# r4dl/StopThePop-Rasterization

Measured on AMD Instinct MI355X. Metric: fwd+bwd frames/sec at 1920×1080, 1M Gaussians; PSNR vs reference, higher is better.
Workload: dtype f32

## Files before the change

stopthepop-rasterization_amd/csrc/stp_render_hier.inc:

```
#include "stp_internal.h"
#include "stp_blend.h"

namespace stp {

#ifdef STP_HIER_STATS
static __device__ unsigned long long g_hier_stats[16];
#if defined(STP_INST_MODE) && STP_INST_MODE == 2 && STP_INST_MID == 8
extern "C" int stp_debug_hier_stats(unsigned long long* out16)
{
    hipError_t e = hipMemcpyFromSymbol(out16, HIP_SYMBOL(g_hier_stats), sizeof(unsigned long long) * 16);
    unsigned long long z[16] = {};
    (void)hipMemcpyToSymbol(HIP_SYMBOL(g_hier_stats), z, sizeof(z));
    return (int)e;
}
#endif
#endif

namespace {

#ifndef STP_BWD_WIN
#define STP_BWD_WIN 256
#endif
#ifndef STP_BWD_RING
#define STP_BWD_RING 512
#endif
#ifndef STP_BWD_WAVES
#define STP_BWD_WAVES 3
#endif
#ifndef STP_FWD_WAVES
#define STP_FWD_WAVES 5
#endif
constexpr int BWD_WIN = STP_BWD_WIN;
constexpr int BWD_RING = STP_BWD_RING;

#ifndef STP_FIFO_GROUPS
#define STP_FIFO_GROUPS 4
#endif
constexpr int FIFO_GROUPS = STP_FIFO_GROUPS;
#ifndef STP_HF_CAP
#define STP_HF_CAP 32
#endif
constexpr int HF_CAP = STP_HF_CAP;

struct HierLds {
    static __host__ __device__ constexpr size_t tail_key() { return 0; }
    static __host__ __device__ constexpr size_t tail_id() { return 16 * 64 * 4; }
    static __host__ __device__ constexpr size_t new_key() { return 2 * 16 * 64 * 4; }
    static __host__ __device__ constexpr size_t new_id() { return 2 * 16 * 64 * 4 + 16 * 32 * 4; }
    static __host__ __device__ constexpr size_t mid_key() { return 2 * 16 * 64 * 4 + 2 * 16 * 32 * 4; }
    static __host__ __device__ constexpr size_t mid_id(int MID) { return mid_key() + 64 * (size_t)MID * 4; }
    static __host__ __device__ constexpr size_t fifo(int MID) { return mid_key() + 2 * 64 * (size_t)MID * 4; }
    static __host__ __device__ constexpr size_t rays(int MID) { return fifo(MID) + 16 * (size_t)FIFO_GROUPS * 16 * 4; }
    static __host__ __device__ constexpr size_t mid_rays(int MID) { return rays(MID) + 4 * 2 * 8 * 4; }
    static __host__ __device__ constexpr size_t fwd_total(int MID) { return mid_rays(MID) + 64 * 4 * 4; }
    static __host__ __device__ constexpr size_t hfifo(int MID) { return fwd_total(MID); }
    static __host__ __device__ constexpr size_t acc(int MID) { return fwd_total(MID); }
    static __host__ __device__ constexpr size_t tag(int MID) { return acc(MID) + 9 * (size_t)BWD_WIN * 8; }
    static __host__ __device__ constexpr size_t dirty(int MID) { return tag(MID) + (size_t)BWD_WIN * 4; }
    static __host__ __device__ constexpr size_t ring(int MID) { return dirty(MID) + (size_t)BWD_WIN * 4; }
    static __host__ __device__ constexpr size_t ring_cs(int MID) { return ring(MID) + (size_t)BWD_RING * 4; }
    static __host__ __device__ constexpr size_t wave_mask(int MID) { return ring_cs(MID) + (size_t)BWD_RING * 4; }
    static __host__ __device__ constexpr size_t total(int MID, int mode) { return mode == 1 ? wave_mask(MID) + 16 : hfifo(MID) + 64 * (size_t)HF_CAP * 4; }
};

__device__ __forceinline__ int hier_remap_tile(int wg, int n_wg)
{
    const int q = n_wg >> 3, r = n_wg & 7;
    const int xcd = wg & 7, k = wg >> 3;
    return (xcd < r ? xcd * (q + 1) : r * (q + 1) + (xcd - r) * q) + k;
}

constexpr int MODE_FWD = 0, MODE_BWD = 1, MODE_FWD_RECORD = 2, MODE_FWD_DEPTH = 3;

template <int HEAD, int MID, bool CULL, int MODE, bool FRCP>
__global__ void __launch_bounds__(256, MODE == MODE_BWD ? STP_BWD_WAVES : (HEAD == 4 && MID == 8 && FRCP) ? STP_FWD_WAVES : 4) render_hier_kernel(const RenderArgs a)
{
    constexpr bool FRESH_QUAD = MODE != MODE_BWD && HEAD == 4 && MID == 8 && FRCP && STP_FWD_WAVES >= 5 && CULL;
    constexpr bool BACKWARD = MODE == MODE_BWD;
    constexpr bool RECORD = MODE == MODE_FWD_RECORD;
    constexpr bool DEPTHVIZ = MODE == MODE_FWD_DEPTH;
    constexpr bool USE_POS = true;
    extern __shared__ __attribute__((aligned(16))) char smem[];
    constexpr int OLDN = (MID - 4) / 4;

    const int lane = (int)(threadIdx.x & 63);
    const int w = __builtin_amdgcn_readfirstlane((int)(threadIdx.x >> 6));
    const int s = lane >> 4;
    const int x = lane & 15;
    const int m = x >> 2;
    const int q = x & 3;

    const int rows = a.ty1 - a.ty0;
    const int t = a.tile_order ? (int)a.tile_order[blockIdx.x] : hier_remap_tile((int)blockIdx.x, a.gx * rows);
    const int tile_x = t % a.gx, tile_y = a.ty0 + t / a.gx;
    const uint2 range = a.ranges[tile_y * a.gx + tile_x];
    if constexpr (BACKWARD) {
        if (a.flag_mode == 1 && a.tile_flags[tile_y * a.gx + tile_x] == 0u) return;
    }

    const int cx = tile_x * TILE + 4 * s, cy = tile_y * TILE + 4 * w;
    const int px = cx + 2 * (m & 1) + (q & 1), py = cy + 2 * (m >> 1) + (q >> 1);
    const bool inside = px < a.W && py < a.H;
    bool active = inside;
    if constexpr (!BACKWARD) {
        if (range.y <= range.x) {
            if (inside) {
                const size_t N = (size_t)a.W * a.H, pid = (size_t)a.W * py + px;
                a.final_T[pid] = 1.0f;
                if constexpr (RECORD) a.n_contrib[pid] = 0u;
                if constexpr (DEPTHVIZ) { a.out_color[pid] = 0.0f; a.out_color[N + pid] = 1.0f; }
                else { a.out_color[pid] = a.bg[0]; a.out_color[N + pid] = a.bg[1]; a.out_color[2 * N + pid] = a.bg[2]; }
            }
            return;
        }
    }
    if constexpr (MODE == MODE_FWD || MODE == MODE_FWD_RECORD) {
        const int n = (int)(range.y - range.x);
        if (a.fused_gather && n <= TS_SMALL) {
            tile_sort_gather_lds(a.gather, reinterpret_cast<uint64_t*>(smem), tile_y * a.gx + tile_x, range, n, (int)threadIdx.x);
            __threadfence_block();
            __syncthreads();
        }
    }

    const int st = w * 4 + s;
    auto fresh_lane = [&]() __attribute__((always_inline)) -> int {
        int l;
        asm volatile("v_mbcnt_lo_u32_b32 %0, -1, 0\n\tv_mbcnt_hi_u32_b32 %0, -1, %0" : "=v"(l));
        return l;
    };
#define STP_ROW_VIEW(L)                                                                                                  \
    const int lrow_ = (L);                                               \
    const int x = lrow_ & 15;                                                                                            \
    const int st_r = w * 4 + (lrow_ >> 4);                                                                               \
    float* const tk = reinterpret_cast<float*>(smem + HierLds::tail_key()) + st_r * 64;                                  \
    int* const ti = reinterpret_cast<int*>(smem + HierLds::tail_id()) + st_r * 64;                                       \
    float* const nk = reinterpret_cast<float*>(smem + HierLds::new_key()) + st_r * 32;                                   \
    int* const ni = reinterpret_cast<int*>(smem + HierLds::new_id()) + st_r * 32;                                        \
    int* const fifo = reinterpret_cast<int*>(smem + HierLds::fifo(MID)) + st_r * FIFO_GROUPS * 16;
    struct QuadView { int q; float* mk; int* mi; int* hfifo; };
#define STP_QUAD_VIEW(L)                                                                                                 \
    const int lquad_ = (L);                                              \
    const int q = lquad_ & 3;                                                                                            \
    const uint32_t qi_ = (uint32_t)(w * 16) + ((uint32_t)lquad_ >> 2);                                                   \
    const uint32_t qmid_ = (MID & (MID - 1)) == 0 ? qi_ << __builtin_ctz(MID) : qi_ * (uint32_t)MID;  \
    float* const mk = reinterpret_cast<float*>(smem + HierLds::mid_key()) + qmid_;                                       \
    int* const mi = reinterpret_cast<int*>(smem + HierLds::mid_id(MID)) + qmid_;                                         \
    float* const mray = reinterpret_cast<float*>(smem + HierLds::mid_rays(MID)) + (qi_ << 2);                            \
    int* const hfifo = reinterpret_cast<int*>(smem + HierLds::hfifo(MID)) + (qi_ << __builtin_ctz(HF_CAP));             \
    const QuadView qv{q, mk, mi, hfifo}; (void)qv; (void)mray;

    const float3 cam = make_float3(a.cam[0], a.cam[1], a.cam[2]);
    const float3 pix_dir = view_ray(a.inv_vp, cam, (float)px, (float)py, a.W, a.H);
    if (q == 0) {
        float* const mray = reinterpret_cast<float*>(smem + HierLds::mid_rays(MID)) + (st * 4 + m) * 4;
        const float3 md = view_ray(a.inv_vp, cam, (float)cx + 0.5f + 2.0f * (float)(m & 1), (float)cy + 0.5f + 2.0f * (float)(m >> 1), a.W, a.H);
        mray[0] = md.x; mray[1] = md.y; mray[2] = md.z; mray[3] = 0.0f;
    }
#define STP_STAGE_VIEW(L)                                                                                                \
    const int lstage_ = (L);                                             \
    const int half = lstage_ >> 5, e = lstage_ & 31;                                                                           \
    const int sxA = tile_x * TILE + 4 * (2 * half), sxB = sxA + 4;                                                       \
    float* const tray = reinterpret_cast<float*>(smem + HierLds::rays(MID)) + (w * 2 + half) * 8;                        \
    float* const nkA = reinterpret_cast<float*>(smem + HierLds::new_key()) + (w * 4 + 2 * half) * 32;                    \
    int* const niA = reinterpret_cast<int*>(smem + HierLds::new_id()) + (w * 4 + 2 * half) * 32;
    {
    STP_STAGE_VIEW(lane)
    if (e == 0) {
        const float3 tA = view_ray(a.inv_vp, cam, (float)sxA + 1.5f, (float)cy + 1.5f, a.W, a.H);
        const float3 tB = view_ray(a.inv_vp, cam, (float)sxB + 1.5f, (float)cy + 1.5f, a.W, a.H);
        tray[0] = tA.x; tray[1] = tA.y; tray[2] = tA.z; tray[3] = 0.0f;
        tray[4] = tB.x; tray[5] = tB.y; tray[6] = tB.z; tray[7] = 0.0f;
    }
    }
    wave_sync();

    unsigned long long* const acc = reinterpret_cast<unsigned long long*>(smem + HierLds::acc(MID));
    int* const tag = reinterpret_cast<int*>(smem + HierLds::tag(MID));
    int* const dirty = reinterpret_cast<int*>(smem + HierLds::dirty(MID));
    int* const ring = reinterpret_cast<int*>(smem + HierLds::ring(MID));
    int* const ring_cs = reinterpret_cast<int*>(smem + HierLds::ring_cs(MID));
    unsigned int* const wave_mask = reinterpret_cast<unsigned int*>(smem + HierLds::wave_mask(MID));
    const float4* const eA = a.entA + range.x;
    const float4* const eB = a.entB + range.x;
    const float4* const eC = a.entC + range.x;
    const float4* const eD = a.entD + range.x;
    const float4* const eF = a.entF + range.x;
    const int list_last = max((int)(range.y - range.x) - 1, 0);
    auto ent_row = [&](const float4* base, int pos) __attribute__((always_inline)) -> float4 {
        return *reinterpret_cast<const float4*>(reinterpret_cast<const char*>(base) + ((uint32_t)pos << 4));
    };
    int staged = 0;
    int ccount = 0;
    auto to_id = [&](int v) __attribute__((always_inline)) -> int {
        if constexpr (!USE_POS) return v;
        else {
            int r = ring[v & (BWD_RING - 1)];
            const bool old = v >= 0 && v < staged - BWD_RING;
            if (__builtin_expect(__any(old), 0)) {
                if (old) r = (int)a.point_list[range.x + min(v, list_last)];
            }
            return v < 0 ? -1 : r;
        }
    };
    if constexpr (BACKWARD) {
        for (int i = (int)threadIdx.x; i < BWD_WIN; i += 256) {
            tag[i] = -1;
            dirty[i] = 0;
#pragma unroll
            for (int k = 0; k < 9; k++) acc[k * BWD_WIN + i] = 0ull;
        }
        __syncthreads();
    }

    char* const log_wave = RECORD ? log_wave_slice(a.blend_log, tile_y * a.gx + tile_x, __builtin_amdgcn_readfirstlane(w), a.log_depth) : nullptr;
    const uint32_t log_cap2 = 2u * (uint32_t)a.log_depth;
    const uint32_t log_lane16 = (uint32_t)lane << LOG_PIECE_SHIFT;
    uint32_t log_j2 = 0u;
    auto log_append = [&](bool upd, int pay) __attribute__((always_inline)) {
        *reinterpret_cast<log_t*>(log_wave + log_record_offset<false>(min(log_j2, log_cap2), log_lane16)) = (log_t)pay;
        log_j2 += upd ? 2u : 0u;
    };
    auto log_records = [&]() __attribute__((always_inline)) -> int { return (int)(log_j2 >> 1); };
    auto log_finish = [&]() __attribute__((always_inline)) {};

    Window<HEAD> head;
    if constexpr (BACKWARD) head.init(); else head.init_padded();
    FwdPixel fp;
    BwdPixel bp;
    if constexpr (BACKWARD) init_bwd_pixel(bp, a, inside, px, py);
    else init_fwd_pixel(fp);

    int n_tail = 0;
    int n_mid = 0;
    int mid_pending = 0;

    float wave_md = 0.0f;
    if constexpr (BACKWARD) {
        wave_md = fmaxf(fmaxf(fabsf(bp.dL_dpix[0]), fabsf(bp.dL_dpix[1])), fabsf(bp.dL_dpix[2]));
#pragma unroll
        for (int off = 32; off > 0; off >>= 1) wave_md = fmaxf(wave_md, __shfl_xor(wave_md, off));
        if (lane == 0) wave_mask[w] = __float_as_uint(wave_md);
        __syncthreads();
        wave_md = fmaxf(fmaxf(__uint_as_float(wave_mask[0]), __uint_as_float(wave_mask[1])),
                        fmaxf(__uint_as_float(wave_mask[2]), __uint_as_float(wave_mask[3])));
        __syncthreads();
    }
    int md_exp = 0;
    if (wave_md > 0.0f && wave_md < 3.0e38f) (void)frexpf(wave_md, &md_exp);
    const double fx_scale = ldexp(1.0, 31 - md_exp), fx_inv = ldexp(1.0, md_exp - 31);
    const float fx_cap = ldexpf(1.0f, min(md_exp + 20, 126));
    auto accumulate = [&](int pos, int id, const float (&g_in)[9]) __attribute__((always_inline)) {
        float g[9];
#pragma unroll
        for (int k = 0; k < 9; k++) g[k] = g_in[k];
        const unsigned long long here = __ballot(1);
        bool mine = true;
        if (((here >> (lane & ~3)) & 0xFull) == 0xFull) {
            const int p0 = quad_bcast_i<0>(pos), p1 = quad_bcast_i<1>(pos), p2 = quad_bcast_i<2>(pos), p3 = quad_bcast_i<3>(pos);
            if (p0 == p1 && p0 == p2 && p0 == p3) {
#pragma unroll
                for (int k = 0; k < 9; k++) {
                    g[k] += __int_as_float(__builtin_amdgcn_mov_dpp(__float_as_int(g[k]), 0xB1, 0xF, 0xF, true));
                    g[k] += __int_as_float(__builtin_amdgcn_mov_dpp(__float_as_int(g[k]), 0x4E, 0xF, 0xF, true));
                }
                mine = q == 0;
            }
        }
        if (!mine) return;
        int cs = -1;
        if (pos >= staged - BWD_RING) cs = ring_cs[pos & (BWD_RING - 1)];
        float gmax = fabsf(g[0]);
#pragma unroll
        for (int k = 1; k < 9; k++) gmax = fmaxf(gmax, fabsf(g[k]));
        if (cs >= 0 && tag[cs] == pos && gmax < fx_cap) {
#pragma unroll
            for (int k = 0; k < 9; k++) {
                const double t = fma((double)g[k], fx_scale, 6755399441055744.0);
                const long long qv = __double_as_longlong(t) - 0x4338000000000000ll;
                atomicAdd(&acc[k * BWD_WIN + cs], (unsigned long long)qv);
            }
            dirty[cs] = 1;
        } else {
#pragma unroll
            for (int k = 0; k < 9; k++) atomicAdd(grad_slot(a, id, k), g[k]);
        }
    };
    auto flush_slot = [&](int cs, int first, int last) __attribute__((always_inline)) {
        if (dirty[cs]) {
            const int old_id = to_id(tag[cs]);
            for (int k = first; k < last; k++) {
                const long long v = (long long)acc[k * BWD_WIN + cs];
                acc[k * BWD_WIN + cs] = 0ull;
                if (v != 0) atomicAdd(grad_slot(a, old_id, k), (float)((double)v * fx_inv));
            }
        }
    };
    auto flush_all = [&]() __attribute__((always_inline)) {
        __syncthreads();
        for (int cs = (int)threadIdx.x; cs < BWD_WIN; cs += 256) flush_slot(cs, 0, 9);
    };

    int front_key = -1;
    float front_col[3] = {0.0f, 0.0f, 0.0f};
    FrontData front_fd{};
    int front_gid = -1;
    auto refresh_front = [&]() __attribute__((always_inline)) {
        if (active && head.num > 0 && head.id[0] != front_key) {
            front_key = head.id[0];
            if constexpr (BACKWARD) {
                front_gid = to_id(front_key);
                front_fd = load_front(a, front_gid);
            } else {
                front_gid = to_id(front_key);
#pragma unroll
                for (int ch = 0; ch < 3; ch++) front_col[ch] = a.features[3 * (size_t)front_gid + ch];
            }
        }
    };
    auto blend_front = [&]() __attribute__((always_inline)) {
        if (!active) { head.num--; return; }
        bool ok;
        if constexpr (BACKWARD) {
            float g[9];
            if (head.id[0] != front_key) refresh_front();
            ok = blend_backward_terms(bp, a, px, py, front_fd, head.store[0], g);
            if (ok) accumulate(head.id[0], front_gid, g);
        } else {
            if (head.id[0] != front_key) refresh_front();
            ok = blend_forward_c(fp, front_col, head.store[0]);
            if constexpr (RECORD) {
                log_append(ok, head.id[0]);
            }
        }
        if (!ok) { active = false; head.num--; return; }
        head.pop();
    };

    float pend_w = 0.0f;
    float pend_c[3] = {0.0f, 0.0f, 0.0f};
    float depth_acc = 0.0f;
    auto pop_forward = [&]() __attribute__((always_inline)) {
#pragma unroll
        for (int ch = 0; ch < 3; ch++) fp.C[ch] = fmaf(pend_w, pend_c[ch], fp.C[ch]);
        const float alpha0 = head.store[0];
        const float test_T = fp.T * (1.0f - alpha0);
        const bool doing = active && !(head.depth[0] < 0.0f);
        const bool upd = doing && !(test_T < T_THRESHOLD);
        const int pay = head.id[0];
        const float4 colr = *reinterpret_cast<const float4*>(reinterpret_cast<const char*>(eF) + ((uint32_t)pay << 4));
        pend_c[0] = colr.x; pend_c[1] = colr.y; pend_c[2] = colr.z;
        pend_w = upd ? alpha0 * fp.T : 0.0f;
        if constexpr (DEPTHVIZ) depth_acc += upd ? head.depth[0] * alpha0 * fp.T : 0.0f;
        fp.T = upd ? test_T : fp.T;
        if constexpr (RECORD) {
            log_append(upd, pay);
        }
        active = active && (upd || !doing);
    };

    auto feed_one = [&](int cid, float3 p0, float3 p1, float3 p2, float4 co, float2 xy) __attribute__((always_inline)) {
        const float depth = depth_along_ray<FRCP>(p0, p1, p2, pix_dir);
        const float dx = xy.x - (float)px, dy = xy.y - (float)py;
        const float power = blend_power(dx, dy, co);
        if constexpr (BACKWARD) {
            if (!active || depth < 0.0f) return;
            if (power > 0.0f) return;
            const float G = exp_blend(power);
            const float alpha = fminf(0.99f, co.w * G);
            if (alpha < ALPHA_THRESHOLD) return;
            head.insert(depth, cid, G);
        } else {
            const float G = exp_blend(power);
            const float alpha = fminf(0.99f, co.w * G);
            const bool pass = active && cid != -1 && !(depth < 0.0f) && !(power > 0.0f) && !(alpha < ALPHA_THRESHOLD);
            head.insert_if(pass, depth, cid, alpha);
        }
    };

    auto feed4_from = [&](const int fid) __attribute__((always_inline)) {
        int pf = 0;
        float4 c0 = make_float4(0, 0, 0, 0), c1 = c0, c2 = c0, co = c0;
        float2 xy = make_float2(0, 0);
        float4 eAq = c0, eBq = c0, eCq = c0, eDq = c0;
        if constexpr (BACKWARD) {
            const int gid_f = to_id(fid);
            if (fid != -1) {
                c0 = a.cov3D_inv[3 * (size_t)gid_f + 0];
                c1 = a.cov3D_inv[3 * (size_t)gid_f + 1];
                c2 = a.cov3D_inv[3 * (size_t)gid_f + 2];
                co = a.conic_opacity[gid_f];
                xy = a.means2D[gid_f];
            }
        } else {
            pf = min(max(fid, 0), list_last);
            eAq = ent_row(eA, pf); eBq = ent_row(eB, pf); eCq = ent_row(eC, pf); eDq = ent_row(eD, pf);
        }
#define STP_FEED(I)                                                                                                     \
    {                                                                                                                   \
                                                                            \
        if constexpr (BACKWARD) { if (head.num >= HEAD) blend_front(); }                                                \
        else pop_forward();                                                                                             \
        const int cid = quad_bcast_i<I>(BACKWARD ? fid : pf);                                                           \
        if constexpr (!BACKWARD) {          \
            if constexpr (I == 0) {                   \
                eDq.w = fid < 0 ? 0.0f : eDq.w;                                                                         \
                dpp_hazard_guard_on(eDq.w);                             \
            } else dpp_hazard_guard();                                                                                  \
            const float depth = depth_along_ray_quad_ent<I, FRCP>(eAq, eBq, eCq, pix_dir);                              \
            const float dx = quad_sub<I>(eCq.y, (float)px), dy = quad_sub<I>(eCq.z, (float)py);                         \
            const float power = blend_power_quad<I>(dx, dy, eDq);                                                       \
            const float alpha = min_099(quad_mul<I>(eDq.w, exp_blend(power)));                                          \
            const bool pass = active && !(depth < 0.0f) && !(power > 0.0f) && !(alpha < ALPHA_THRESHOLD);               \
            head.replace_front(pass, pass ? depth : -FLT_MAX, cid, alpha);                                              \
        } else if (cid != -1) {                                                                                         \
            const float3 b0 = make_float3(quad_bcast<I>(c0.x), quad_bcast<I>(c0.y), quad_bcast<I>(c0.z));               \
            const float3 b1 = make_float3(quad_bcast<I>(c1.x), quad_bcast<I>(c1.y), quad_bcast<I>(c1.z));               \
            const float3 b2 = make_float3(quad_bcast<I>(c2.x), quad_bcast<I>(c2.y), quad_bcast<I>(c2.z));               \
            const float4 bco = make_float4(quad_bcast<I>(co.x), quad_bcast<I>(co.y), quad_bcast<I>(co.z), quad_bcast<I>(co.w)); \
            const float2 bxy = make_float2(quad_bcast<I>(xy.x), quad_bcast<I>(xy.y));                                   \
            feed_one(cid, b0, b1, b2, bco, bxy);                                                                        \
        }                                                                                                               \
// ... 491 lines not shown
```

stopthepop-rasterization_amd/csrc/stp_tilesort.h:

```cpp
#pragma once

#include "stp_device.h"

namespace stp {

constexpr int TS_SMALL = 1024;

struct EntryGather {
    uint64_t* keys;
    uint32_t* point_list;
    const float4* gpack;
    const float* features;
    int gx;
    int cull_mask;
    float4* entA; float4* entB; float4* entC; float4* entD; float4* entF;
};

__device__ __forceinline__ void write_entry(const EntryGather& a, size_t i, int id, int tile)
{
    const float4* __restrict__ gp = a.gpack + 4 * (size_t)id;
    const float4 pa = gp[0], pb = gp[1], pc = gp[2], pd = gp[3];
    const float3 col = make_float3(a.features[3 * (size_t)id], a.features[3 * (size_t)id + 1], a.features[3 * (size_t)id + 2]);
    a.entA[i] = pa;
    a.entB[i] = pb;
    a.entC[i] = make_float4(pc.x, pc.y, pc.z, __int_as_float(id));
    a.entD[i] = pd;
    float spare = 0.0f;
    if (a.cull_mask) spare = __uint_as_float(subtile_mask(a.cull_mask, pd, make_float2(pc.y, pc.z), tile % a.gx, tile / a.gx));
    a.entF[i] = make_float4(col.x, col.y, col.z, spare);
}

__device__ __forceinline__ void tile_sort_gather_lds(const EntryGather& a, uint64_t* s_key, int tile, uint2 range, int n, int tid)
{
    uint64_t* const keys = a.keys + range.x;
    uint32_t* const list = a.point_list + range.x;
    int m = 2;
    while (m < n) m <<= 1;
    const uint64_t tile_bits = keys[0] & 0xFFFFFFFF00000000ull;
    for (int i = tid; i < m; i += 256) {
        s_key[i] = i < n ? ((keys[i] << 32) | list[i]) : ~0ull;
    }
    __syncthreads();
    for (int k = 2; k <= m; k <<= 1)
        for (int j = k >> 1; j > 0; j >>= 1) {
            for (int c = tid; c < (m >> 1); c += 256) {
                const int lo = ((c & ~(j - 1)) << 1) | (c & (j - 1));
                const int hi = lo | j;
                const bool up = (lo & k) == 0;
                const uint64_t x = s_key[lo], y = s_key[hi];
                if ((x > y) == up) { s_key[lo] = y; s_key[hi] = x; }
            }
            const int j_next = j > 1 ? (j >> 1) : k;
            const bool last = j == 1 && k == m;
            if (j > 64 || j_next > 64 || last) __syncthreads();
            else wave_sync();
        }
    for (int i = tid; i < n; i += 256) {
        const uint64_t k = s_key[i];
        const int id = (int)(uint32_t)k;
        keys[i] = tile_bits | (k >> 32);
        list[i] = (uint32_t)id;
        if (a.gpack) write_entry(a, (size_t)range.x + i, id, tile);
    }
}

}
```

stopthepop-rasterization_amd/csrc/stp_tilesort.hip:

```cpp
#include "stp_internal.h"
#include "stp_device.h"
#include "stp_tilesort.h"
#include <rocprim/block/block_radix_sort.hpp>

namespace stp {

namespace {

constexpr int TS_CAP = 4096;
#ifndef STP_GATHER_WAVES
#define STP_GATHER_WAVES 6
#endif

struct TileSortArgs {
    const uint2* ranges;
    uint64_t* keys_scratch;
    uint32_t* list_scratch;
    int id_passes;
    int tile0;
    const uint32_t* tile_order;
    EntryGather e;
};

template <int IPT> struct TileRadix {
    using Sort = rocprim::block_radix_sort<uint32_t, 256, IPT, uint32_t>;
    template <class WriteEntry>
    static __device__ __forceinline__ void run(typename Sort::storage_type& st, uint64_t* keys, uint32_t* list, int n, int tid, WriteEntry&& write_entry_at)
    {
        const uint64_t tile_bits = keys[0] & 0xFFFFFFFF00000000ull;
        uint32_t k[IPT], v[IPT];
#pragma unroll
        for (int j = 0; j < IPT; j++) {
            const int i = tid * IPT + j;
            k[j] = i < n ? (uint32_t)keys[i] : 0xFFFFFFFFu;
            v[j] = i < n ? list[i] : 0xFFFFFFFFu;
        }
        __syncthreads();
        Sort().sort_to_striped(k, v, st, 0, 32);
#pragma unroll
        for (int j = 0; j < IPT; j++) {
            const int i = j * 256 + tid;
            if (i < n) {
                keys[i] = tile_bits | k[j];
                list[i] = v[j];
                write_entry_at(i, (int)v[j]);
            }
        }
    }
};

template <int CAP, int MIN_N>
__global__ void __launch_bounds__(256, (CAP == TS_SMALL ? STP_GATHER_WAVES : 4)) tile_sort_gather_kernel(const TileSortArgs a)
{
    using Radix8 = TileRadix<8>;
    using Radix16 = TileRadix<16>;
    constexpr size_t RADIX_BYTES = CAP == TS_CAP ? (sizeof(typename Radix16::Sort::storage_type) > sizeof(typename Radix8::Sort::storage_type) ? sizeof(typename Radix16::Sort::storage_type) : sizeof(typename Radix8::Sort::storage_type)) : 0;
    constexpr size_t RAW_BYTES = RADIX_BYTES > sizeof(uint64_t) * CAP ? RADIX_BYTES : sizeof(uint64_t) * CAP;
    __shared__ __attribute__((aligned(16))) char s_raw[RAW_BYTES];
    uint64_t* const s_key = reinterpret_cast<uint64_t*>(s_raw);
    static_assert(CAP != TS_CAP || RAW_BYTES >= sizeof(int) * 13 * 256, "the long-segment path keeps its counters in the sort's LDS area");
    const int tid = (int)threadIdx.x;
    const int n_wg = (int)gridDim.x, wg = (int)blockIdx.x;
    const int xq = n_wg >> 3, xr = n_wg & 7, xcd = wg & 7;
    const int tile = a.tile0 + (a.tile_order ? (int)a.tile_order[wg] : (xcd < xr ? xcd * (xq + 1) : xr * (xq + 1) + (xcd - xr) * xq) + (wg >> 3));
    const uint2 range = a.ranges[tile];
    const int n = (int)(range.y - range.x);
    if (n <= MIN_N || (CAP == TS_SMALL && n > TS_SMALL)) return;
    uint64_t* const keys = a.e.keys + range.x;
    uint32_t* const list = a.e.point_list + range.x;

    if constexpr (CAP == TS_CAP) {
        if (n <= CAP && a.id_passes == 0) {
            auto we = [&](int i, int id) __attribute__((always_inline)) { if (a.e.gpack) write_entry(a.e, (size_t)range.x + i, id, tile); };
            if (n <= 2048) Radix8::run(*reinterpret_cast<typename Radix8::Sort::storage_type*>(s_raw), keys, list, n, tid, we);
            else Radix16::run(*reinterpret_cast<typename Radix16::Sort::storage_type*>(s_raw), keys, list, n, tid, we);
            return;
        }
    }
    if (n <= CAP) {
        tile_sort_gather_lds(a.e, s_key, tile, range, n, tid);
        return;
    }

    if constexpr (CAP == TS_SMALL) return;
    int* const s_hist = reinterpret_cast<int*>(s_raw);
    int* const s_wcnt = s_hist + 256;
    int* const s_hall = s_hist + 5 * 256;
    uint64_t* src_k = keys; uint32_t* src_v = list;
    uint64_t* dst_k = a.keys_scratch + range.x; uint32_t* dst_v = a.list_scratch + range.x;
    const int n_pass = a.id_passes + 4;
    const int wv = tid >> 6, ln = tid & 63;
    const unsigned long long lt_mask = (1ull << ln) - 1ull;
    int done_passes = 0;
    for (int i = tid; i < 8 * 256; i += 256) s_hall[i] = 0;
    __syncthreads();
    {
        const int n4 = n & ~1023;
        for (int i0 = 0; i0 < n; i0 += 1024) {
            uint64_t k[4]; uint32_t v[4]; bool ok[4];
#pragma unroll
            for (int r = 0; r < 4; r++) { const int i = i0 + 256 * r + tid; ok[r] = i0 < n4 || i < n; k[r] = ok[r] ? src_k[i] : 0ull; v[r] = (ok[r] && a.id_passes) ? src_v[i] : 0u; }
#pragma unroll
            for (int r = 0; r < 4; r++)
                if (ok[r]) {
                    for (int p = 0; p < a.id_passes; p++) atomicAdd(&s_hall[256 * p + (int)((v[r] >> (8 * p)) & 0xFF)], 1);
#pragma unroll
                    for (int p = 0; p < 4; p++) atomicAdd(&s_hall[256 * (a.id_passes + p) + (int)((k[r] >> (8 * p)) & 0xFF)], 1);
                }
        }
    }
    __syncthreads();
    for (int pass = 0; pass < n_pass; pass++) {
        const bool on_id = pass < a.id_passes;
        const int shift = 8 * (on_id ? pass : pass - a.id_passes);
        auto digit = [&](uint64_t k, uint32_t v) __attribute__((always_inline)) { return (int)(((on_id ? (uint64_t)v : k) >> shift) & 0xFF); };
        s_hist[tid] = s_hall[256 * pass + tid];
#pragma unroll
        for (int r = 0; r < 4; r++) s_wcnt[256 * r + tid] = 0;
        __syncthreads();
        const bool same = s_hist[digit(src_k[0], src_v[0])] == n;
        __syncthreads();
        if (same) continue;
        if (tid < 64) {
            int c[4], sum = 0;
#pragma unroll
            for (int k = 0; k < 4; k++) { c[k] = s_hist[4 * tid + k]; sum += c[k]; }
            int inc = sum;
#pragma unroll
            for (int o = 1; o < 64; o <<= 1) { const int v = __shfl_up(inc, o); if (tid >= o) inc += v; }
            int run = inc - sum;
#pragma unroll
            for (int k = 0; k < 4; k++) { s_hist[4 * tid + k] = run; run += c[k]; }
        }
        __syncthreads();
        for (int c0 = 0; c0 < n; c0 += 4 * 256) {
            uint64_t k[4]; uint32_t v[4]; int d[4], rank[4]; bool valid[4];
#pragma unroll
            for (int r = 0; r < 4; r++) {
                const int i = c0 + 256 * r + tid;
                valid[r] = i < n;
                k[r] = 0; v[r] = 0;
                if (valid[r]) { k[r] = src_k[i]; v[r] = src_v[i]; }
            }
#pragma unroll
            for (int r = 0; r < 4; r++) {
                d[r] = valid[r] ? digit(k[r], v[r]) : 0;
                unsigned long long peers = __ballot(valid[r]);
#pragma unroll
                for (int bit = 0; bit < 8; bit++) {
                    const bool one = ((d[r] >> bit) & 1) != 0;
                    const unsigned long long bal = __ballot(one);
                    peers &= one ? bal : ~bal;
                }
                rank[r] = __popcll(peers & lt_mask);
                if (valid[r] && rank[r] == 0) atomicAdd(&s_wcnt[256 * r + d[r]], __popcll(peers) << (8 * wv));
            }
            __syncthreads();
            auto fields = [](unsigned int wc) __attribute__((always_inline)) { return (int)((wc & 0xFFu) + ((wc >> 8) & 0xFFu) + ((wc >> 16) & 0xFFu) + (wc >> 24)); };
#pragma unroll
            for (int r = 0; r < 4; r++) {
                if (valid[r]) {
                    int below = 0;
#pragma unroll
                    for (int rr = 0; rr < 4; rr++)
                        if (rr < r) below += fields((unsigned int)s_wcnt[256 * rr + d[r]]);
                    const unsigned int wc = (unsigned int)s_wcnt[256 * r + d[r]];
                    below += (int)((wv > 0 ? (wc & 0xFFu) : 0u) + (wv > 1 ? ((wc >> 8) & 0xFFu) : 0u) + (wv > 2 ? ((wc >> 16) & 0xFFu) : 0u));
                    const int at = s_hist[d[r]] + below + rank[r];
                    dst_k[at] = k[r];
                    dst_v[at] = v[r];
                }
            }
            __syncthreads();
            {
                int tot = 0;
#pragma unroll
                for (int r = 0; r < 4; r++) {
                    const unsigned int wc = (unsigned int)s_wcnt[256 * r + tid];
                    if (wc != 0u) { tot += fields(wc); s_wcnt[256 * r + tid] = 0; }
                }
                s_hist[tid] += tot;
            }
            __syncthreads();
        }
        uint64_t* tk = src_k; src_k = dst_k; dst_k = tk;
        uint32_t* tv = src_v; src_v = dst_v; dst_v = tv;
        done_passes++;
        __threadfence_block();
        __syncthreads();
    }
    if (done_passes & 1) {
        for (int i = tid; i < n; i += 256) { keys[i] = src_k[i]; list[i] = src_v[i]; }
        __threadfence_block();
        __syncthreads();
    }
    if (a.e.gpack) {
#pragma unroll 4
        for (int i = tid; i < n; i += 256) write_entry(a.e, (size_t)range.x + i, (int)list[i], tile);
    }
}

}

hipError_t launch_tile_sort_gather(const FrameParams& f, const GeometryState& g, const BinningState& b, const ImageState& img, int R, bool unordered, hipStream_t st)
{
    if (R <= 0) return hipSuccess;
    TileSortArgs a{};
    a.id_passes = 0;
    if (unordered)
        for (unsigned int top = (unsigned int)(f.P > 1 ? f.P - 1 : 1); top; top >>= 8) a.id_passes++;
    a.ranges = img.ranges; a.e.keys = b.keys; a.e.point_list = b.point_list; a.keys_scratch = b.keys_unsorted; a.list_scratch = b.point_list_unsorted;
    const bool entries = f.s.sort_mode == MODE_HIER || f.s.sort_mode == MODE_KBUFFER;
    a.e.gpack = entries ? g.gpack : nullptr;
    a.e.features = f.colors_precomp ? f.colors_precomp : g.rgb;
    a.e.gx = f.gx;
    a.tile0 = f.gx * f.ty0;
    a.e.cull_mask = subtile_mask_kind(f.s);
    const int gmode = (tile_order_used(f) && !unordered) ? gather_order_mode() : 0;
    a.tile_order = gmode == 1 ? img.tile_counts + f.gx * f.ty0 : gmode == 2 ? img.tile_cursor + f.gx * f.ty0 : nullptr;
    a.e.entA = b.entA; a.e.entB = b.entB; a.e.entC = b.entC; a.e.entD = b.entD; a.e.entF = b.entF;
    const int n_tiles = f.gx * (f.ty1 - f.ty0);
    if (n_tiles <= 0) return hipSuccess;
    if (!f.fused_gather) hipLaunchKernelGGL((tile_sort_gather_kernel<TS_SMALL, 0>), dim3(n_tiles), dim3(256), 0, st, a);
    hipLaunchKernelGGL((tile_sort_gather_kernel<TS_CAP, TS_SMALL>), dim3(n_tiles), dim3(256), 0, st, a);
    return hipGetLastError();
}

}
```

Measured before the change: 453.6.

## Replace LDS bitonic sort for small tiles with register-resident lane-shuffle network

Small per-tile segments (up to 1024 entries) are now sorted with a bitonic network that keeps keys in registers. Intra-wave stages use DPP, swizzle and permlane swaps, and only cross-wave stages go through double-buffered LDS. This applies both in the fused forward gather path and in the small-cap tile sort kernel. It aims to cut LDS traffic and barriers per compare stage, at the cost of more registers, doubled LDS for the small kernel, and reliance on gfx950 permlane swap intrinsics.

```diff
diff --git a/stopthepop-rasterization_amd/csrc/stp_render_hier.inc b/stopthepop-rasterization_amd/csrc/stp_render_hier.inc
--- a/stopthepop-rasterization_amd/csrc/stp_render_hier.inc
+++ b/stopthepop-rasterization_amd/csrc/stp_render_hier.inc
@@ -117,7 +117,8 @@
     if constexpr (MODE == MODE_FWD || MODE == MODE_FWD_RECORD) {
         const int n = (int)(range.y - range.x);
         if (a.fused_gather && n <= TS_SMALL) {
-            tile_sort_gather_lds(a.gather, reinterpret_cast<uint64_t*>(smem), tile_y * a.gx + tile_x, range, n, (int)threadIdx.x);
+            static_assert(HierLds::fwd_total(MID) >= (size_t)TS_SMALL_LDS_BYTES, "the sort's exchange buffers fit in the forward's carve");
+            tile_sort_gather_regs(a.gather, reinterpret_cast<uint64_t*>(smem), tile_y * a.gx + tile_x, range, n, (int)threadIdx.x);
             __threadfence_block();
             __syncthreads();
         }
diff --git a/stopthepop-rasterization_amd/csrc/stp_tilesort.h b/stopthepop-rasterization_amd/csrc/stp_tilesort.h
--- a/stopthepop-rasterization_amd/csrc/stp_tilesort.h
+++ b/stopthepop-rasterization_amd/csrc/stp_tilesort.h
@@ -5,6 +5,7 @@
 namespace stp {
 
 constexpr int TS_SMALL = 1024;
+constexpr int TS_SMALL_LDS_BYTES = 2 * TS_SMALL * 8;
 
 struct EntryGather {
     uint64_t* keys;
@@ -64,4 +65,164 @@
     }
 }
 
-}
+
+template <int X> __device__ __forceinline__ uint32_t lane_xor_u32(uint32_t v)
+{
+    static_assert(X == 1 || X == 2 || X == 4 || X == 8, "");
+    if constexpr (X == 1) return (uint32_t)__builtin_amdgcn_mov_dpp((int)v, 0xB1, 0xF, 0xF, true);
+    else if constexpr (X == 2) return (uint32_t)__builtin_amdgcn_mov_dpp((int)v, 0x4E, 0xF, 0xF, true);
+    else if constexpr (X == 4) return (uint32_t)__builtin_amdgcn_ds_swizzle((int)v, 0x101F);
+    else return (uint32_t)__builtin_amdgcn_mov_dpp((int)v, 0x128, 0xF, 0xF, true);
+}
+template <int X> __device__ __forceinline__ uint64_t lane_xor_u64(uint64_t v)
+{
+    return ((uint64_t)lane_xor_u32<X>((uint32_t)(v >> 32)) << 32) | lane_xor_u32<X>((uint32_t)v);
+}
+template <int B> __device__ __forceinline__ void lane_bit_transpose(uint64_t& a, uint64_t& b)
+{
+    static_assert(B == 4 || B == 5, "");
+    uint32_t al = (uint32_t)a, ah = (uint32_t)(a >> 32), bl = (uint32_t)b, bh = (uint32_t)(b >> 32);
+    if constexpr (B == 5) {
+        const auto l = __builtin_amdgcn_permlane32_swap(al, bl, false, false), h = __builtin_amdgcn_permlane32_swap(ah, bh, false, false);
+        al = l[0]; bl = l[1]; ah = h[0]; bh = h[1];
+    } else {
+        const auto l = __builtin_amdgcn_permlane16_swap(al, bl, false, false), h = __builtin_amdgcn_permlane16_swap(ah, bh, false, false);
+        al = l[0]; bl = l[1]; ah = h[0]; bh = h[1];
+    }
+    a = ((uint64_t)ah << 32) | al;
+    b = ((uint64_t)bh << 32) | bl;
+}
+__device__ __forceinline__ void compare_exchange(uint64_t& lo, uint64_t& hi, bool up)
+{
+    const uint64_t x = lo, y = hi;
+    const bool sw = (x > y) == up;
+    lo = sw ? y : x;
+    hi = sw ? x : y;
+}
+__device__ __forceinline__ uint64_t compare_keep(uint64_t mine, uint64_t p, bool keep_min)
+{
+    return ((mine > p) == keep_min) ? p : mine;
+}
+
+template <int KPL, int JB, class Up> __device__ __forceinline__ void regs_stage(uint64_t (&key)[KPL], int lane, Up&& up)
+{
+    if constexpr (JB <= 3) {
+        const bool lower = ((lane >> JB) & 1) == 0;
+        uint64_t p[KPL];
+#pragma unroll
+        for (int q = 0; q < KPL; q++) p[q] = lane_xor_u64<(1 << JB)>(key[q]);
+#pragma unroll
+        for (int q = 0; q < KPL; q++) key[q] = compare_keep(key[q], p[q], lower == up(q >> 1, (q & 1) != 0));
+    } else if constexpr (JB <= 5) {
+        const bool bit6 = ((lane >> JB) & 1) != 0;
+#pragma unroll
+        for (int h = 0; h < KPL / 2; h++) {
+            lane_bit_transpose<JB>(key[2 * h], key[2 * h + 1]);
+            compare_exchange(key[2 * h], key[2 * h + 1], up(h, bit6));
+            lane_bit_transpose<JB>(key[2 * h], key[2 * h + 1]);
+        }
+    } else if constexpr (JB == 6) {
+#pragma unroll
+        for (int h = 0; h < KPL / 2; h++) compare_exchange(key[2 * h], key[2 * h + 1], up(h, false));
+    } else {
+        static_assert(JB == 7 && KPL == 4, "");
+        compare_exchange(key[0], key[2], up(0, false));
+        compare_exchange(key[1], key[3], up(0, true));
+    }
+}
+template <int KPL, int JB, class Up> __device__ __forceinline__ void regs_merge_from(uint64_t (&key)[KPL], int lane, Up&& up)
+{
+    regs_stage<KPL, JB>(key, lane, up);
+    if constexpr (JB > 0) regs_merge_from<KPL, JB - 1>(key, lane, up);
+}
+
+template <int KPL> __device__ __forceinline__ void regs_network(uint64_t (&key)[KPL], uint64_t* s_key, int n, int m, int tid)
+{
+    constexpr int WAVE_KEYS = 64 * KPL, WB = KPL == 2 ? 7 : 8;
+    const int lane = lane_id();
+    const int wb = __builtin_amdgcn_readfirstlane(tid >> 6) * WAVE_KEYS;
+    auto all_padding = [&]() __attribute__((always_inline)) -> bool {
+        bool any = false;
+#pragma unroll
+        for (int q = 0; q < KPL; q++) any |= key[q] != ~0ull;
+        return __builtin_amdgcn_ballot_w64(any) == 0ull;
+    };
+    if (wb < n) {
+#define STP_TS_LEVEL(KB)                                                                                                 \
+        if ((1 << KB) <= m) {                                                                                            \
+            const bool up_l = ((lane >> KB) & 1) == 0;                                                                   \
+            regs_merge_from<KPL, KB - 1>(key, lane, [&](int, bool bit6) __attribute__((always_inline)) { return KB == 6 ? !bit6 : up_l; }); \
+        }
+        STP_TS_LEVEL(1) STP_TS_LEVEL(2) STP_TS_LEVEL(3) STP_TS_LEVEL(4) STP_TS_LEVEL(5) STP_TS_LEVEL(6)
+#undef STP_TS_LEVEL
+    }
+    int buf = 0;
+    for (int kb = 7; (1 << kb) <= m; kb++) {
+        auto up = [&](int h, bool) __attribute__((always_inline)) { return (((wb + 128 * h) >> kb) & 1) == 0; };
+        for (int jb = kb - 1; jb >= WB; jb--) {
+            uint64_t* const s = s_key + buf * TS_SMALL;
+            buf ^= 1;
+#pragma unroll
+            for (int q = 0; q < KPL; q++) s[wb + 64 * q + lane] = key[q];
+            __syncthreads();
+            const bool keep_min = (((wb >> jb) & 1) == 0) == up(0, false);
+#pragma unroll
+            for (int q = 0; q < KPL; q++) key[q] = compare_keep(key[q], s[(wb ^ (1 << jb)) + 64 * q + lane], keep_min);
+        }
+        if (all_padding()) continue;
+        if constexpr (KPL == 4) {
+            if (kb > 7) regs_stage<KPL, 7>(key, lane, up);
+        }
+        regs_merge_from<KPL, 6>(key, lane, up);
+    }
+}
+
+__device__ __forceinline__ void tile_sort_gather_regs(const EntryGather& a, uint64_t* s_key, int tile, uint2 range, int n, int tid)
+{
+    uint64_t* const keys = a.keys + range.x;
+    uint32_t* const list = a.point_list + range.x;
+    int m = 2;
+    while (m < n) m <<= 1;
+    const int kpl = m > 512 ? 4 : 2;
+    const int i0 = __builtin_amdgcn_readfirstlane(tid >> 6) * 64 * kpl + lane_id();
+    uint64_t key[4];
+    const uint32_t tile_hi = (uint32_t)(keys[0] >> 32);
+#pragma unroll
+    for (int q = 0; q < 4; q++) {
+        const int i = i0 + 64 * q;
+        key[q] = ~0ull;
+        if (q < kpl && i < n) key[q] = (keys[i] << 32) | list[i];
+    }
+    if (kpl == 4) regs_network<4>(key, s_key, n, m, tid);
+    else {
+        uint64_t key2[2] = {key[0], key[1]};
+        regs_network<2>(key2, s_key, n, m, tid);
+        key[0] = key2[0]; key[1] = key2[1];
+    }
+    if (n <= 256) {
+        uint64_t* const s = s_key + TS_SMALL;
+        if (i0 < n) s[i0] = key[0];
+        if (i0 + 64 < n) s[i0 + 64] = key[1];
+        __syncthreads();
+        if (tid < n) {
+            const uint64_t k = s[tid];
+            const int id = (int)(uint32_t)k;
+            keys[tid] = ((uint64_t)tile_hi << 32) | (k >> 32);
+            list[tid] = (uint32_t)id;
+            if (a.gpack) write_entry(a, (size_t)range.x + tid, id, tile);
+        }
+        return;
+    }
+#pragma unroll 1
+    for (int q = 0; q < kpl; q++) {
+        const int i = i0 + 64 * q;
+        if (i >= n) break;
+        const uint64_t k = q == 0 ? key[0] : q == 1 ? key[1] : q == 2 ? key[2] : key[3];
+        const int id = (int)(uint32_t)k;
+        keys[i] = ((uint64_t)tile_hi << 32) | (k >> 32);
+        list[i] = (uint32_t)id;
+        if (a.gpack) write_entry(a, (size_t)range.x + i, id, tile);
+    }
+}
+
+}
diff --git a/stopthepop-rasterization_amd/csrc/stp_tilesort.hip b/stopthepop-rasterization_amd/csrc/stp_tilesort.hip
--- a/stopthepop-rasterization_amd/csrc/stp_tilesort.hip
+++ b/stopthepop-rasterization_amd/csrc/stp_tilesort.hip
@@ -55,7 +55,8 @@
     using Radix8 = TileRadix<8>;
     using Radix16 = TileRadix<16>;
     constexpr size_t RADIX_BYTES = CAP == TS_CAP ? (sizeof(typename Radix16::Sort::storage_type) > sizeof(typename Radix8::Sort::storage_type) ? sizeof(typename Radix16::Sort::storage_type) : sizeof(typename Radix8::Sort::storage_type)) : 0;
-    constexpr size_t RAW_BYTES = RADIX_BYTES > sizeof(uint64_t) * CAP ? RADIX_BYTES : sizeof(uint64_t) * CAP;
+    constexpr size_t KEY_BYTES = CAP == TS_SMALL ? (size_t)TS_SMALL_LDS_BYTES : sizeof(uint64_t) * CAP;
+    constexpr size_t RAW_BYTES = RADIX_BYTES > KEY_BYTES ? RADIX_BYTES : KEY_BYTES;
     __shared__ __attribute__((aligned(16))) char s_raw[RAW_BYTES];
     uint64_t* const s_key = reinterpret_cast<uint64_t*>(s_raw);
     static_assert(CAP != TS_CAP || RAW_BYTES >= sizeof(int) * 13 * 256, "the long-segment path keeps its counters in the sort's LDS area");
@@ -78,7 +79,8 @@
         }
     }
     if (n <= CAP) {
-        tile_sort_gather_lds(a.e, s_key, tile, range, n, tid);
+        if constexpr (CAP == TS_SMALL) tile_sort_gather_regs(a.e, s_key, tile, range, n, tid);
+        else tile_sort_gather_lds(a.e, s_key, tile, range, n, tid);
         return;
     }
 
```

Result: no change. 457.0 (median of 6 runs) (+0.8%).
